# YukunXia/VLOAM-CMU-16833

Measured on AMD Instinct MI355X. Metric: scans/sec end-to-end odometry on 64x2048 cloud, higher is better.
Workload: dtype f32 points / f64 poses+residuals; 1 GPU; configs[2]: scanRegistration + laserOdometry + laserMapping scan-to-map ICP (voxel-hash local map, ~200 scans), synthetic HDL-64E 64x2048; sequences=1, map_warmup_sweeps=200, map_points_at_last_sweep=119454

## Files before the change

vloam-cmu-16833_amd/__init__.py:

```python
import os as _os
_os.environ.setdefault("GPU_MAX_HW_QUEUES", "16")
import ctypes as C
import os
import numpy as np

_DIR = os.path.dirname(os.path.abspath(__file__))
LIB_PATH = os.environ.get("VLOAM_HIP_LIB") or os.path.join(_DIR, "libvloam_hip.so")

VLOAM_OK, ERR_INVALID, ERR_HIP, ERR_CAPACITY, ERR_EMPTY, ERR_NO_DEVICE, ERR_ORDER = 0, -1, -2, -3, -4, -5, -6

K_MAX_RINGS, K_SECTORS = 64, 6
K_MAX_SHARP, K_MAX_LESS_SHARP, K_MAX_FLAT = 768, 7680, 1536
K_MAX_LO_FACTORS = K_MAX_SHARP + K_MAX_FLAT
K_IMG_MAX_CORNERS = 1024
K_LM_MAX_TRACE = 104
K_STACK_CAP_CORNER, K_STACK_CAP_SURF = 8192, 24576
K_MAP_FACTOR_CAP = K_STACK_CAP_CORNER + K_STACK_CAP_SURF


class VloamError(RuntimeError):
    def __init__(self, status, msg):
        super().__init__("vloam status %d: %s" % (status, msg))
        self.status = status

# ... 900 lines not shown
        if q_wmap_wodom is not None:
            opt.q_wmap_wodom[:] = [float(v) for v in q_wmap_wodom]
        if t_wmap_wodom is not None:
            opt.t_wmap_wodom[:] = [float(v) for v in t_wmap_wodom]
        return opt

    @staticmethod
    def _import_result(out):
        return {k: (out[0][k].copy() if out[0][k].ndim else out[0][k].item()) for k in MAP_IMPORT_RESULT_DTYPE.names if k != "pad"}

    def map_import(self, corner, surf, q_wmap_wodom=None, t_wmap_wodom=None):
        opt = self._import_options(q_wmap_wodom, t_wmap_wodom)
        c, s = self._cloud_arg(corner), self._cloud_arg(surf)
        out = np.zeros(1, dtype=MAP_IMPORT_RESULT_DTYPE)
        self._chk(self.L.vloam_map_import(self.h, C.byref(opt), c[1], C.c_longlong(c[2]), s[1], C.c_longlong(s[2]), _fp(out)))
        return self._import_result(out)

    def map_import_device(self, corner, surf, q_wmap_wodom=None, t_wmap_wodom=None):
        import torch
        opt = self._import_options(q_wmap_wodom, t_wmap_wodom)
        ptr, n = [None, None], [0, 0]
        for k, c in enumerate((corner, surf)):
            if c is not None and c.shape[0] > 0:
                assert c.is_cuda and c.is_contiguous() and c.dtype == torch.float32 and c.shape[-1] == 4
                ptr[k], n[k] = C.c_void_p(c.data_ptr()), int(c.shape[0])
        res = torch.zeros(MAP_IMPORT_RESULT_DTYPE.itemsize, dtype=torch.uint8, device=next((c.device for c in (corner, surf) if c is not None), "cuda"))
        self._chk(self.L.vloam_map_import_device(self.h, C.byref(opt), ptr[0], C.c_longlong(n[0]), ptr[1], C.c_longlong(n[1]), C.c_void_p(res.data_ptr())))
        return self._import_result(res.cpu().numpy().view(MAP_IMPORT_RESULT_DTYPE))

    def published_map(self):
        n, f = C.c_longlong(0), C.c_int(-1)
        self._chk(self.L.vloam_get_published_map(self.h, None, C.c_longlong(0), C.byref(n), C.byref(f)))
        buf = np.zeros((max(n.value, 1), 4), dtype=np.float32)
        self._chk(self.L.vloam_get_published_map(self.h, _fp(buf), C.c_longlong(n.value), C.byref(n), C.byref(f)))
        return buf[:n.value], f.value

    def published_cloud(self):
        n, f = C.c_int(0), C.c_int(-1)
        self._chk(self.L.vloam_get_published_cloud(self.h, None, 0, C.byref(n), C.byref(f)))
        buf = np.zeros((max(n.value, 1), 4), dtype=np.float32)
        self._chk(self.L.vloam_get_published_cloud(self.h, _fp(buf), n.value, C.byref(n), C.byref(f)))
        return buf[:n.value], f.value

    def published_device_ptr(self, which):
        p, n, f = C.c_void_p(), C.c_longlong(0), C.c_int(-1)
        self._chk(self.L.vloam_published_device_ptr(self.h, int(which), C.byref(p), C.byref(n), C.byref(f)))
        return p.value, n.value, f.value

    def map_health(self):
        v = self.debug_raw(2, 69, np.int32)
        return dict(keys=(int(v[0]), int(v[4])), purged=(int(v[1]), int(v[5])), block_keys=(int(v[2]), int(v[6])), rebuilds=int(v[8]),
                    max_candidates=int(v[9]), deferred=(int(v[10]), int(v[11])))

    def map_force_rebuild(self):
        n = C.c_longlong(0)
        self._chk(self.L.vloam_debug_get(self.h, 2, 70, None, C.c_longlong(0), C.byref(n)))

    def map_force_grow(self):
        n = C.c_longlong(0)
        self._chk(self.L.vloam_debug_get(self.h, 2, 74, None, C.c_longlong(0), C.byref(n)))

    def map_dump(self, kind):
        rows = self.debug_raw(2, 67 + kind, np.uint32, max_bytes=1 << 30).reshape(-1, 7)
        return rows[:, 2].astype(np.int32), rows[:, 3:7].copy().view(np.float32)


def _same_cloud(given, own):
    a = np.ascontiguousarray(given, dtype=np.float32).reshape(-1, 4)
    return a.shape == own.shape and np.array_equal(a.view(np.uint32), np.ascontiguousarray(own).view(np.uint32))


class ScanRegistration:

    def __init__(self, handle):
        self.hd = handle

    def init(self):
        pass

    def reset(self):
        self.hd.reset_frame()

    def input(self, laserCloudIn):
        self.hd.scan_registration(laserCloudIn)

    def output(self):
        return tuple(self.hd.features(k) for k in range(5))


class LaserOdometry:

    def __init__(self, handle):
        self.hd = handle
        self._pose = None

    def init(self):
        pass

    def input(self, *clouds):
        if not clouds:
            return
        if len(clouds) != 5:
            raise TypeError("LaserOdometry.input takes the five clouds of ScanRegistration.output")
        edits = {}
        for k, (name, c) in enumerate(zip(("laserCloud", "cornerPointsSharp", "cornerPointsLessSharp", "surfPointsFlat", "surfPointsLessFlat"), clouds)):
            if not _same_cloud(c, self.hd.features(k)):
# ... 81 lines not shown
```

vloam-cmu-16833_amd/csrc/map_kernels.h:

```cpp
#pragma once
#include <hip/hip_runtime.h>
#include <vector>
#include "../../include/vloam_hip/c_api.h"
#include "sr_kernels.h"
#include "vloam_device.h"

namespace vloam {

constexpr int kCubeW = 21, kCubeH = 21, kCubeD = 11, kCubeNum = kCubeW * kCubeH * kCubeD;
constexpr int kStackCapCorner = 8192;
constexpr int kStackCapSurf = 24576;
constexpr int kMapFactorCap = kStackCapCorner + kStackCapSurf;
constexpr int kStackCapSurfStep = 8192, kStackCapSurfMax = 131072;
static_assert(kStackCapSurfMax <= (1 << 17), "the tier's raw-point arrival stamp keeps 17 bits of stack index (k_map_finalize_tier)");
constexpr int kPendCap = 16;
__host__ __device__ inline int vox_radix(float inv) { return (int)(50.0f * inv) + 4; }

struct __attribute__((aligned(32))) VoxelRec {
  unsigned long long key;
  float sx, sy, sz, si;
  int count;
  int pend_cnt;
};
static_assert(sizeof(VoxelRec) == 32, "one voxel, one half cache line");

struct VoxelTable {
  VoxelRec* rec;
  int* pend;
  unsigned mask;
  ulonglong2* blk;
  unsigned bslots_mask;
  int* stats;
  __host__ __device__ void rebase(size_t off) { rbp(rec, off); rbp(pend, off); rbp(blk, off); rbp(stats, off); }
};
constexpr int kMaxProbe = 128;
constexpr int kCandChunk = 256;
constexpr int kCandCache = 128;

constexpr int kDsMaxBins = 256;
constexpr int kDsBinTarget = 512;
constexpr int kDsBinCap = 4096;
constexpr int kDsBigCell = 32;
constexpr int kDsBigCap = 128;

struct DsScratch {
  unsigned long long* region;
  unsigned long long* over;
  unsigned long long* tmp;
  unsigned long long* sorted;
  unsigned long long* splitters;
  int* cursor;
  unsigned long long* done;
  int stack_cap;
  __host__ __device__ void rebase(size_t off) {
    rbp(region, off); rbp(over, off); rbp(tmp, off); rbp(sorted, off); rbp(splitters, off); rbp(cursor, off); rbp(done, off);
  }
};

struct StackInfo {
  int n_stack[2];
  int error;
};

struct MapFrame {
  int n_uniq[2];
  int n_stack[2];
  int n_touched[2];
  int n_deferred[2];
  int n_newraw[2];
  int rolled;
  int error;
  int n_factors[2][2];
  int max_candidates;
  int fallback_solves;
};

constexpr int kPubBuckets = 2 * kCubeNum;
constexpr int kPubLdsKeys = 4096;
constexpr long long kPubMapCapDefault = 2097152, kPubMapCapMin = 256, kPubMapCapMax = 16777216;
struct PubHeader { long long n; int overflow; int pad; };
struct MapPub {
  int pub_number = 0;
  int skip_n = 1;
  bool due(int frame_count) const { return ((long long)frame_count * skip_n) % pub_number == 0; }
  long long cap = 0;
  int cloud_on = 0;
  int* cnt = nullptr;
  int* off = nullptr;
  int* cur = nullptr;
  unsigned long long* keys = nullptr;
  float4* vals = nullptr;
  float4* out[2] = {nullptr, nullptr};
  PubHeader* hdr[2] = {nullptr, nullptr};
  float4* cloud[2] = {nullptr, nullptr};
  int* cloud_n[2] = {nullptr, nullptr};
  hipEvent_t ev_map[2] = {nullptr, nullptr}, ev_cloud[2] = {nullptr, nullptr};
  int map_seq = 0, cloud_seq = 0;
  int map_frame[2] = {-1, -1}, cloud_frame[2] = {-1, -1};
  int mapped = 0;
  void rebase(size_t o) {
    rbp(cnt, o); rbp(off, o); rbp(cur, o); rbp(keys, o); rbp(vals, o);
    for (int k = 0; k < 2; k++) { rbp(out[k], o); rbp(hdr[k], o); rbp(cloud[k], o); rbp(cloud_n[k], o); }
  }
};

struct MapGrow {
  int max_log2 = 28;
  int lg[2] = {0, 0};
  long long steps = 0;
  long long inc_rec[2] = {0, 0};
  long long inc_blk[2] = {0, 0};
  unsigned long long* progress = nullptr;
  long long step_at[2] = {-1, -1};
  static constexpr int kEvRing = 4;
  hipEvent_t ev_prog[kEvRing] = {};
  int failed_log2 = 0;
  struct Retired { void* p[3]; hipEvent_t ev; };
  std::vector<Retired> retired;
  std::vector<void*> leftover;
};

struct LocAux { int shift[3]; int si_error; double guess[7]; };
struct MapLocalize {
  char* base = nullptr;
  MapState* state = nullptr;
  MapFrame* frame = nullptr;
  LocAux* aux = nullptr;
// ... 12 lines not shown
};

struct MapContext {
  MapState* state = nullptr;
  MapFrame* frame = nullptr;
  VoxelTable tab[2];
  int* cube_cnt = nullptr;
  DsScratch ds[2];
  unsigned ds_gen = 0;
  static constexpr int kSets = kBufferSets;
  float4* stack_sets[kSets][2] = {};
  StackInfo* stack_info[kSets] = {};
  float4* stack[2] = {nullptr, nullptr};
  float4* stack_map[2] = {nullptr, nullptr};
  int* touched[2] = {nullptr, nullptr};
  int* deferred[2] = {nullptr, nullptr};
  int* newraw[2] = {nullptr, nullptr};
  FactorTable F[2];
  LMRecord* rec = nullptr;
  int surf_cap = kStackCapSurf;
  int factor_cap() const { return kStackCapCorner + surf_cap; }
  bool tier() const { return surf_cap > kStackCapSurf; }
  float4* nbr = nullptr;
  int4* cbox = nullptr;
  float4* ccand = nullptr;
  VoxelRec* rebuild_tmp = nullptr;
  int rebuild_cap = 0;
  int* rebuild_n = nullptr;
  int* host_flags = nullptr;
  int rebuild_cooldown[kMaxBatch][2] = {};
  long long rebuilds = 0;
  MapGrow* grow = nullptr;
  Sess se;
  int sel = 0;
  MapContext for_session(int b) const {
    MapContext m = *this;
    const size_t off = (size_t)b * se.ss;
    rbp(m.state, off); rbp(m.frame, off); m.tab[0].rebase(off); m.tab[1].rebase(off); rbp(m.cube_cnt, off); m.ds[0].rebase(off); m.ds[1].rebase(off);
    for (int c = 0; c < kSets; c++) { rbp(m.stack_sets[c][0], off); rbp(m.stack_sets[c][1], off); rbp(m.stack_info[c], off); }
    for (int k = 0; k < 2; k++) { rbp(m.stack[k], off); rbp(m.stack_map[k], off); rbp(m.touched[k], off); rbp(m.deferred[k], off); rbp(m.newraw[k], off); m.F[k].rebase(off); }
    rbp(m.rec, off); rbp(m.nbr, off); rbp(m.cbox, off); rbp(m.ccand, off); rbp(m.registered, off); rbp(m.assoc_cyc, off); rbp(m.ts_log, off); rbp(m.rebuild_tmp, off); rbp(m.rebuild_n, off);
    if (m.host_flags) m.host_flags += 2 * b;
    m.pub.rebase(off);
    m.se.B = 1; m.sel = 0;
    return m;
  }
  MapLocalize* loc = nullptr;
  MapPub pub;
  float4* registered = nullptr;
  long long* assoc_cyc = nullptr;
  long long* ts_log = nullptr;
  int max_points = 0;
  float inv_leaf[2] = {0, 0};
};

vloam_status map_layout(MapContext* m, const vloam_config& cfg, Arena& A);
vloam_status map_init(MapContext* m, hipStream_t st);
vloam_status map_enqueue(MapContext* m, const vloam_config& cfg, hipStream_t st, const SRBuffers& cur, LOState* lo, double* traj_row14,
                         bool skip_frame, int set, ProfHook* ph, hipEvent_t done = nullptr);
vloam_status map_force_rebuild(MapContext* m, hipStream_t st);
void map_destroy(MapContext* m);
vloam_status map_stack_enqueue(MapContext* m, hipStream_t st, const SRBuffers& cur, int set, ProfHook* ph, hipEvent_t done = nullptr);
vloam_status map_get_cloud(MapContext* m, hipStream_t st, int which, const SRBuffers& cur, float* xyzi4, int cap, int* n);
vloam_status map_export(MapContext* m, hipStream_t st, float* xyzi4, long long cap, long long* n);
vloam_status map_export_kind(MapContext* m, hipStream_t st, int kind, float* xyzi4, long long cap, long long* n);
bool map_publishes(const MapContext* m, bool skip_frame);
vloam_status map_publish_enqueue(MapContext* m, hipStream_t st, const float4* cloud, const FrameScalars* S, int frame, bool skip_frame, ProfHook* ph,
                                 hipEvent_t done);
vloam_status map_published_get(MapContext* m, int which, float* xyzi4, long long cap, long long* n, int* frame, void** d_ptr);
vloam_status map_error(MapContext* m, int* err_bits, int clear_mask = 0, long long* fallback_solves = nullptr);
vloam_status map_debug_get(MapContext* m, int item, void* buf, long long cap, long long* n);
vloam_status map_counts(MapContext* m, long long c[16]);
vloam_status map_query_enqueue(MapContext* m, hipStream_t st, int kind, int k, float radius, const void* d_xyz_pad4, int n, void* d_xyzi4, void* d_d2,
                               void* d_count);
vloam_status map_score_enqueue(MapContext* m, hipStream_t st, const void* d_corner, int n_corner, const void* d_surf, int n_surf, const int stride[2],
                               const float radius[2], const double* d_q4t3, int M, void* d_out);
vloam_status map_localize_alloc(MapContext* m, hipStream_t st);
void map_localize_free(MapContext* m);
vloam_status map_localize_enqueue(MapContext* m, hipStream_t st, const float4* corner, int n_corner, const float4* surf, int n_surf, int set,
                                  const double* row7, const double pose7[7], int pose_frame, vloam_localize_result* d_result);
void map_loc_prepare_launch(hipStream_t st, const MapContext* m, const StackInfo* si, const double* row7, const double pose7[7], int pose_frame);
void map_loc_finish_launch(hipStream_t st, const MapContext* m, vloam_localize_result* d_result);
void map_stack_enqueue_loc(MapContext* m, hipStream_t st, const float4* corner, const float4* surf);
vloam_status map_import_run(MapContext* m, hipStream_t st, const double pose7[7], const void* const cloud[2], const int n[2], bool host_clouds,
                            vloam_map_import_result* h_result);
vloam_status map_force_grow(MapContext* m, hipStream_t st);
void map_grow_release(MapContext* m);
vloam_status map_grow_init(MapContext* m, hipStream_t st);
void map_grow_destroy(MapContext* m);
vloam_status map_grow_rehash(MapContext* m, hipStream_t st, int kind);
vloam_status map_grow_before_sweep(MapContext* m, hipStream_t st);
void map_grow_progress_enqueue(MapContext* m, hipStream_t st);
vloam_status map_ckpt_pack(MapContext* m, hipStream_t st, long long n_rec[2], VoxelRec** d_out, float ms[2]);
vloam_status map_ckpt_unpack(MapContext* m, hipStream_t st, const void* recs, const long long n_rec[2], float* ms);
int map_grow_restore_log2(const MapContext* m, int kind, long long live, long long blk);
vloam_status map_grow_restore(MapContext* m, hipStream_t st, const int lg[2], const long long live[2], const long long blk[2], long long mapped);

}
```

vloam-cmu-16833_amd/csrc/map_kernels.hip:

```cpp
#include <hip/hip_runtime.h>
#include <math.h>
#include <string.h>
#include <type_traits>
#include "lm_solve.h"
#include "map_kernels.h"
#include "map_device.h"
#include "map_table.h"
#include "subwave.h"

namespace vloam {

__device__ void map_purge(const VoxelTable& T, const MapState* ms, int first, int stride) {
  const int cW = ms->cenW, cH = ms->cenH, cD = ms->cenD;
  int dead = 0;
  for (unsigned s = (unsigned)first; s <= T.mask; s += (unsigned)stride) {
    const RecVal v = rec_load(&T.rec[s]);
    if (v.key == 0 || v.count == 0) continue;
    int Ai, Aj, Ak;
    unpack_cube(v.key, &Ai, &Aj, &Ak);
    const int i = Ai + cW, j = Aj + cH, kk = Ak + cD;
    if (i < 0 || i >= kCubeW || j < 0 || j >= kCubeH || kk < 0 || kk >= kCubeD) { rec_store_value(&T.rec[s], make_float4(0.f, 0.f, 0.f, 0.f), 0, 0); dead++; }
  }
  if (dead) atomicAdd(&T.stats[1], dead);
}
// ... 13 lines not shown
  const double emin = q + 2.0 * p * cos(phi + 2.0943951023931954923);
  *e_max = emax;
  *e_mid = 3.0 * q - emax - emin;
  const double r0[3] = {A[0][0] - emax, A[0][1], A[0][2]}, r1[3] = {A[0][1], A[1][1] - emax, A[1][2]}, r2[3] = {A[0][2], A[1][2], A[2][2] - emax};
  const double c0[3] = {r0[1] * r1[2] - r0[2] * r1[1], r0[2] * r1[0] - r0[0] * r1[2], r0[0] * r1[1] - r0[1] * r1[0]};
  const double c1[3] = {r0[1] * r2[2] - r0[2] * r2[1], r0[2] * r2[0] - r0[0] * r2[2], r0[0] * r2[1] - r0[1] * r2[0]};
  const double c2[3] = {r1[1] * r2[2] - r1[2] * r2[1], r1[2] * r2[0] - r1[0] * r2[2], r1[0] * r2[1] - r1[1] * r2[0]};
  const double n0 = c0[0] * c0[0] + c0[1] * c0[1] + c0[2] * c0[2], n1 = c1[0] * c1[0] + c1[1] * c1[1] + c1[2] * c1[2],
               n2 = c2[0] * c2[0] + c2[1] * c2[1] + c2[2] * c2[2];
  const bool u0 = n0 >= n1 && n0 >= n2, u1 = !u0 && n1 >= n2;
  const double nn = u0 ? n0 : (u1 ? n1 : n2);
  const double inv = 1.0 / sqrt(nn);
#pragma unroll
  for (int k = 0; k < 3; k++) v[k] = (u0 ? c0[k] : (u1 ? c1[k] : c2[k])) * inv;
}

__device__ bool householder_ls_5x3(double* A, double* b, double* x) {
  const int m = 5, n = 3;
  for (int k = 0; k < n; k++) {
    double nrm = 0;
    for (int i = k; i < m; i++) nrm += A[i * n + k] * A[i * n + k];
    nrm = sqrt(nrm);
    if (nrm == 0.0) return false;
    const double alpha = (A[k * n + k] > 0) ? -nrm : nrm;
    const double v0 = A[k * n + k] - alpha;
    double vtv = v0 * v0;
    for (int i = k + 1; i < m; i++) vtv += A[i * n + k] * A[i * n + k];
    if (vtv != 0.0) {
      for (int j = k + 1; j < n; j++) {
        double s = v0 * A[k * n + j];
        for (int i = k + 1; i < m; i++) s += A[i * n + k] * A[i * n + j];
        s = 2.0 * s / vtv;
        A[k * n + j] -= s * v0;
        for (int i = k + 1; i < m; i++) A[i * n + j] -= s * A[i * n + k];
      }
      double s = v0 * b[k];
      for (int i = k + 1; i < m; i++) s += A[i * n + k] * b[i];
      s = 2.0 * s / vtv;
      b[k] -= s * v0;
      for (int i = k + 1; i < m; i++) b[i] -= s * A[i * n + k];
    }
    A[k * n + k] = alpha;
    for (int i = k + 1; i < m; i++) A[i * n + k] = 0.0;
  }
  for (int k = n - 1; k >= 0; k--) {
    double s = b[k];
    for (int j = k + 1; j < n; j++) s -= A[k * n + j] * x[j];
    if (A[k * n + k] == 0.0) return false;
    x[k] = s / A[k * n + k];
  }
  return true;
}

template <int G, int KB>
__global__ __launch_bounds__(256) __attribute__((amdgpu_waves_per_eu(5))) void k_map_assoc(const float4* __restrict__ stack0, const float4* __restrict__ stack1, VoxelTable T0,
                                                   VoxelTable T1, float inv0, float inv1, const MapState* __restrict__ ms, MapFrame* fr,
                                                   float4* __restrict__ nbr, int outer, int4* __restrict__ cbox, float4* __restrict__ ccand,
                                                   long long* __restrict__ dbg_cyc , size_t ss) {
  VL_SESSION(ss); RB(stack0); RB(stack1); T0.rebase(so_); T1.rebase(so_); RB(ms); RB(fr); RB(nbr); RB(cbox); RB(ccand); RB(dbg_cyc);
  long long tp[8] = {0, 0, 0, 0, 0, 0, 0, 0};
  if (dbg_cyc) tp[0] = clock64();
  constexpr int Q = 64 / G, QW = 4 * Q;
  constexpr int U = G == 16 ? 4 : 2, CH = U * G;
  static_assert(CH <= kCandCache, "the second round's candidate cache holds kCandCache entries per slot");
  const int lane = threadIdx.x & 63, wave = threadIdx.x >> 6, gl = lane & (G - 1), qi = wave * Q + lane / G;
  const int nc = ms->n_corner_stack, nsf = ms->n_surf_stack;
  const int wc = (nc + QW - 1) / QW, ws = (nsf + QW - 1) / QW, cpc = (wc + 7) >> 3, cps = (ws + 7) >> 3;
  const int bq = (int)blockIdx.x >> 3, xcd = (int)blockIdx.x & 7;
  if (bq >= cpc + cps || !ms->do_optimize) return;
  const int kind = bq < cpc ? 0 : 1;
  const int i = (kind ? xcd * cps + (bq - cpc) : xcd * cpc + bq) * QW + qi;
  const bool live = i < (kind ? nsf : nc);
  if (__ballot(live) == 0ull) return;
  const int slot = kind ? kStackCapCorner + i : i;
  const VoxelTable T = kind ? T1 : T0;
  const float inv = kind ? inv1 : inv0;
  const unsigned nv = (unsigned)vox_radix(inv);
  __shared__ u64 s_cand[QW][CH + 8];
  __shared__ u64 s_bestk[QW][8];
  __shared__ float4 s_bestp[QW][8];
  __shared__ int s_piece[QW][3][8];
  __shared__ int s_np[QW][4];
  constexpr int kRawCap = 64;
  __shared__ u64 s_rawk[QW][kRawCap];
  __shared__ int s_rawn[QW][kRawCap];
  __shared__ int s_nraw[QW];
  float4 pointOri = make_float4(0.f, 0.f, 0.f, 0.f);
  int4 box0 = make_int4(0, 0, 0, 0), box1 = make_int4(0, 0, -1, 0);
  if (live) {
    pointOri = kind ? stack1[i] : stack0[i];
    if (outer > 0) { box0 = cbox[2 * slot]; box1 = cbox[2 * slot + 1]; }
  }
  const float4 sel = associate_to_map(pointOri, ms->parameters, ms->parameters + 4);
  const float q0 = sel.x, q1 = sel.y, q2 = sel.z;
  const int cen0 = ms->cenW, cen1 = ms->cenH, cen2 = ms->cenD;
  const int ctr0 = ms->centerCube[0] - cen0, ctr1 = ms->centerCube[1] - cen1, ctr2 = ms->centerCube[2] - cen2;
  const float mg = outer == 0 ? 1.051f : 1.001f;
  int blo0 = (int)floorf((q0 - mg) * inv), bhi0 = (int)floorf((q0 + mg) * inv);
  int blo1 = (int)floorf((q1 - mg) * inv), bhi1 = (int)floorf((q1 + mg) * inv);
  int blo2 = (int)floorf((q2 - mg) * inv), bhi2 = (int)floorf((q2 + mg) * inv);
  bool from_cache = false;
  int total = 0;
  if (outer > 0 && live) {
    const int4 b0 = box0, b1 = box1;
    from_cache = b1.z >= 0 && b1.z <= kCandCache && b0.x <= blo0 && b0.y >= bhi0 && b0.z <= blo1 && b0.w >= bhi1 && b1.x <= blo2 && b1.y >= bhi2;
    if (from_cache) total = b1.z;
  }
  const bool search = live && !from_cache;
  bool chain_too_long = false;
  if (dbg_cyc) tp[1] = clock64() + (__float_as_int(q0) & 0) + (total & 0);
  if (gl < 8) s_bestk[qi][gl] = ~0ull;
  if (gl < 4) s_np[qi][gl] = 0;
  if (gl == 4) s_nraw[qi] = 0;
  sw_lds_sync();
  if (__ballot(search) != 0ull) {
    if (search && gl < 3) {
      const int lo = gl == 0 ? blo0 : (gl == 1 ? blo1 : blo2), hi = gl == 0 ? bhi0 : (gl == 1 ? bhi1 : bhi2);
      const int ctr = gl == 0 ? ctr0 : (gl == 1 ? ctr1 : ctr2), cen = gl == 0 ? cen0 : (gl == 1 ? cen1 : cen2);
      const int halfw = gl == 2 ? 1 : 2, wdim = gl == 0 ? kCubeW : (gl == 1 ? kCubeH : kCubeD);
      const double leaf = 1.0 / (double)inv;
      const int Amin = cube_lo((double)lo * leaf), Amax = cube_hi((double)(hi + 1) * leaf);
      int n = 0;
      bool ovf = false;
      for (int A = Amin; A <= Amax; A++) {
        if (abs(A - ctr) > halfw) continue;
        const int wv = A + cen;
        if (wv < 0 || wv >= wdim) continue;
        const int base = cube_voxel_base(A, inv);
        const int ia = max(lo, base + 1), ib = min(hi, cube_voxel_base(A + 1, inv) + 1);
        if (ia > ib) continue;
        for (int blk = (ia - base) >> 2; blk <= ((ib - base) >> 2); blk++) {
          if ((unsigned)blk > (unsigned)(kVoxMax >> 2) || n >= 8) { ovf = true; break; }
          int m4 = 0;
#pragma unroll
          for (int t = 0; t < 4; t++) { const int iv = base + (blk << 2) + t; if (iv >= ia && iv <= ib) m4 |= 1 << t; }
          s_piece[qi][gl][n] = ((A + 8192) << 11) | (blk << 4) | m4;
          n++;
        }
      }
      s_np[qi][gl] = n;
      if (ovf) s_np[qi][3] = 1;
    }
    sw_lds_sync();
  }
// ... 167 lines not shown
    }
    if (__ballot(from_cache && act) != 0ull) {
      float4 cc[U];
#pragma unroll
      for (int u = 0; u < U; u++) {
        const int w = c0 + gl + u * G;
        cc[u] = make_float4(0.f, 0.f, 0.f, __uint_as_float(0xffffffffu));
        if (from_cache && act && w < total) cc[u] = ccand[(size_t)slot * kCandCache + w];
      }
#pragma unroll
      for (int u = 0; u < U; u++) {
        const unsigned tie = __float_as_uint(cc[u].w);
        const float d0 = q0 - cc[u].x, d1 = q1 - cc[u].y, d2 = q2 - cc[u].z;
        const u64 k = ((u64)__float_as_uint(d0 * d0 + d1 * d1 + d2 * d2) << 32) | tie;
        if (from_cache && tie != 0xffffffffu) { key_u[u] = k; px[u] = cc[u].x; py[u] = cc[u].y; pz[u] = cc[u].z; }
      }
    }
    if (dbg_cyc && c0 == 0) tp[4] = clock64() + ((int)key_u[0] & 0);
    select_rounds(act, c0 > 0);
    if (dbg_cyc && c0 == 0) tp[5] = clock64();
  }
  const int nraw = min(s_nraw[qi], kRawCap);
  const bool raw_overflow = s_nraw[qi] > kRawCap;
  if (__ballot(live && nraw > 0) != 0ull) {
    int total_raw = 0;
    for (c0 = 0;; c0 += CH) {
      const bool act = live && nraw > 0 && (c0 == 0 || c0 < total_raw);
      if (__ballot(act) == 0ull) break;
      reset_candidates();
      int produced = 0;
      for (int r0 = 0; __ballot(act && r0 < nraw) != 0ull; r0 += G) {
        const int r = r0 + gl;
        const int nr = (act && r < nraw) ? s_rawn[qi][r] : 0;
        const u64 vk = (act && r < nraw) ? s_rawk[qi][r] : 0ull;
        const int inc = grp_scan_incl<G>(nr);
        const int tot = grp_sum<G>(nr);
        int o = produced + inc - nr;
        for (int j = 1; j <= nr; j++, o++)
          if (o >= c0 && o < c0 + CH) s_cand[qi][o - c0] = key_with_seq(vk, j);
        produced += tot;
      }
      if (act) total_raw = produced;
      sw_lds_sync();
      ncand = act ? min(total_raw - c0, CH) : 0;
      probe_pair(std::integral_constant<int, 0>{});
      if constexpr (U > 2) { if (__ballot(2 * G < ncand) != 0ull) probe_pair(std::integral_constant<int, 2>{}); }
      select_rounds(act, true);
    }
  }
  if (outer == 0 && search && gl == 0) {
    cbox[2 * slot] = make_int4(blo0, bhi0, blo1, bhi1);
    cbox[2 * slot + 1] = make_int4(blo2, bhi2, (total <= kCandCache && !overflow && s_nraw[qi] == 0) ? total : -1, total);
  }
  if (live && gl < 5) {
    const u64 k4 = s_bestk[qi][4];
    const bool ok = k4 != ~0ull && __uint_as_float((unsigned)(k4 >> 32)) < 1.0f;
    float4 p = s_bestp[qi][gl];
    p.w = ok ? 1.0f : 0.0f;
    nbr[slot * 5 + gl] = p;
  }
  if (live && gl == 0 && total > kCandChunk) atomicMax(&fr->max_candidates, total);
  if (__ballot(chain_too_long || (live && overflow)) && lane == 0) atomicOr(&fr->error, kErrMapFull);
  if (__ballot(live && raw_overflow) && lane == 0) atomicOr(&fr->error, kErrMapDeferred);
  if (dbg_cyc && lane == 0) {
    tp[6] = clock64();
    if (tp[3] == 0) tp[3] = tp[2];
    if (tp[4] == 0) tp[4] = tp[3];
    for (int k = 0; k < 6; k++) atomicAdd((unsigned long long*)&dbg_cyc[outer * 8 + k], (unsigned long long)(tp[k + 1] - tp[k]));
    atomicAdd((unsigned long long*)&dbg_cyc[outer * 8 + 7], 1ull);
  }
}

#define VL_MAP_TIER 0
#define VL_MAP_KERNEL(name) name
#define VL_MAP_CAP_PARAM
#define VL_MAP_SURF_CAP kStackCapSurf
#define VL_MAP_FACTOR_CAP kMapFactorCap
#include "map_prepare_fit.inc.h"
#define VL_MAP_TIER 1
#define VL_MAP_KERNEL(name) name##_tier
#define VL_MAP_CAP_PARAM , int surf_cap
#define VL_MAP_SURF_CAP surf_cap
#define VL_MAP_FACTOR_CAP F.cap
#include "map_prepare_fit.inc.h"

__device__ void map_update(MapState* ms, double* traj_row14) {
  const double* q = ms->q_wodom_curr;
  const double n2 = q[0] * q[0] + q[1] * q[1] + q[2] * q[2] + q[3] * q[3];
  double qi[4] = {0, 0, 0, 0};
  if (n2 > 0.0) { qi[0] = -q[0] / n2; qi[1] = -q[1] / n2; qi[2] = -q[2] / n2; qi[3] = q[3] / n2; }
  double r[4], t[3];
  dquat_mul(ms->parameters, qi, r);
  for (int k = 0; k < 4; k++) ms->q_wmap_wodom[k] = r[k];
  dquat_rot(ms->q_wmap_wodom, ms->t_wodom_curr, t);
  for (int k = 0; k < 3; k++) ms->t_wmap_wodom[k] = ms->parameters[4 + k] - t[k];
  if (traj_row14) for (int k = 0; k < 7; k++) traj_row14[7 + k] = ms->parameters[k];
}

__device__ bool map_put_raw_point(const VoxelTable& T, u64 voxel_key, int seq, float4 p, int stamp) {
  const u64 key = key_with_seq(voxel_key, seq);
  unsigned s = (unsigned)mix64(key) & T.mask;
  for (int probe = 0; probe < kMaxProbe; probe++, s = (s + 1) & T.mask) {
    const u64 old = atomicCAS(&T.rec[s].key, 0ull, key);
    if (old == 0ull || old == key) {
      if (old == 0ull) atomicAdd(&T.stats[0], 1);
      rec_store_value(&T.rec[s], p, 1, stamp);
      return true;
    }
  }
  return false;
}
__device__ void map_drop_raw_points(const VoxelTable& T, u64 voxel_key, int n) {
// ... 252 lines not shown
}

vloam_status map_layout(MapContext* m, const vloam_config& cfg, Arena& A) {
  bool ok = true;
  ok = ok && A.take(&m->state, 1) && A.take(&m->frame, 1) && A.take(&m->cube_cnt, 2 * (size_t)kCubeNum);
  const int lg = cfg.map_capacity_log2 < 10 ? 10 : (cfg.map_capacity_log2 > 28 ? 28 : cfg.map_capacity_log2);
  const size_t slots = (size_t)1 << lg;
  for (int k = 0; k < 2 && ok; k++) {
    VoxelTable& T = m->tab[k];
    if (m->grow) { T.rec = nullptr; T.pend = nullptr; T.blk = nullptr; ok = ok && A.take(&T.stats, 4); }
    else ok = ok && A.take(&T.rec, slots) && A.take(&T.pend, slots * kPendCap) && A.take(&T.stats, 4);
    T.mask = (unsigned)(slots - 1);
    const size_t bslots = slots / 2;
    if (!m->grow) ok = ok && A.take(&T.blk, bslots);
    T.bslots_mask = (unsigned)(bslots - 1);
    DsScratch& D = m->ds[k];
    if (k == 0) for (int c = 0; c < MapContext::kSets; c++) ok = ok && A.take(&m->stack_info[c], 1);
    D.stack_cap = k ? m->surf_cap : kStackCapCorner;
    ok = ok && A.take(&D.region, (size_t)kDsMaxBins * kDsBinCap) && A.take(&D.over, (size_t)cfg.max_points) && A.take(&D.tmp, (size_t)cfg.max_points) &&
         A.take(&D.sorted, (size_t)cfg.max_points) && A.take(&D.splitters, (size_t)kDsMaxBins) && A.take(&D.cursor, (size_t)kDsMaxBins + 4) &&
         A.take(&D.done, (size_t)kDsMaxBins);
    for (int c = 0; c < MapContext::kSets; c++) ok = ok && A.take(&m->stack_sets[c][k], (size_t)D.stack_cap);
    m->stack[k] = m->stack_sets[0][k];
    ok = ok && A.take(&m->stack_map[k], (size_t)D.stack_cap) && A.take(&m->touched[k], (size_t)D.stack_cap) && A.take(&m->deferred[k], (size_t)D.stack_cap) &&
         A.take(&m->newraw[k], (size_t)D.stack_cap);
    FactorTable& F = m->F[k];
    F.cap = m->factor_cap();
    ok = ok && A.take(&F.type, (size_t)F.cap) && A.take(&F.p, 3 * (size_t)F.cap) && A.take(&F.A, 3 * (size_t)F.cap) && A.take(&F.B, 3 * (size_t)F.cap) &&
         A.take(&F.resid, 3 * (size_t)F.cap) && A.take(&F.ctype, (size_t)F.cap) && A.take(&F.cslot, (size_t)F.cap) && A.take(&F.cpack, 11 * (size_t)F.cap) && A.take(&F.dg, 8 * (size_t)F.cap) &&
         A.take(&F.rowcnt, (size_t)F.cap / 64 + 1);
    if (m->tier()) F.rowmask = nullptr;
    else ok = ok && A.take(&F.rowmask, (size_t)F.cap / 64 + 2);
    F.gsync = nullptr;
    F.err = ok ? &m->frame->error : nullptr;
    F.fallbacks = ok ? &m->frame->fallback_solves : nullptr;
    F.host_degraded = nullptr;
    F.gen = 0; F.spin_limit = 1 << 18;
  }
  ok = ok && A.take(&m->rec, 2) && A.take(&m->nbr, 5 * (size_t)m->factor_cap());
  ok = ok && A.take(&m->cbox, 2 * (size_t)m->factor_cap()) && A.take(&m->ccand, (size_t)m->factor_cap() * kCandCache);
  m->rebuild_cap = m->grow ? 0 : (int)(slots / 2);
  if (m->grow) { m->rebuild_tmp = nullptr; m->grow->lg[0] = m->grow->lg[1] = lg; ok = ok && A.take(&m->rebuild_n, 2); }
  else ok = ok && A.take(&m->rebuild_tmp, (size_t)m->rebuild_cap) && A.take(&m->rebuild_n, 2);
  ok = ok && A.take(&m->registered, (size_t)cfg.max_points) && A.take(&m->assoc_cyc, 16) && A.take(&m->ts_log, 2048);
  MapPub& P = m->pub;
  if (P.pub_number > 0) {
    ok = ok && A.take(&P.cnt, (size_t)kPubBuckets) && A.take(&P.off, (size_t)kPubBuckets + 1) && A.take(&P.cur, (size_t)kPubBuckets) &&
         A.take(&P.keys, (size_t)P.cap) && A.take(&P.vals, (size_t)P.cap);
    for (int k = 0; k < 2; k++) ok = ok && A.take(&P.out[k], (size_t)P.cap) && A.take(&P.hdr[k], 1);
  }
  if (P.cloud_on) for (int k = 0; k < 2; k++) ok = ok && A.take(&P.cloud[k], (size_t)cfg.max_points) && A.take(&P.cloud_n[k], 1);
  if (!ok) return VLOAM_ERR_HIP;
  m->max_points = cfg.max_points;
  m->inv_leaf[0] = 1.0f / cfg.mapping_line_resolution;
  m->inv_leaf[1] = 1.0f / cfg.mapping_plane_resolution;
  return VLOAM_OK;
}

vloam_status map_init(MapContext* m, hipStream_t st) {
  if (m->grow && map_grow_init(m, st) != VLOAM_OK) return VLOAM_ERR_HIP;
  if (!m->host_flags) {
    if (hipHostMalloc((void**)&m->host_flags, sizeof(int) * 2 * kMaxBatch, hipHostMallocMapped) != hipSuccess) { m->host_flags = nullptr; return VLOAM_ERR_HIP; }
    for (int k = 0; k < 2 * kMaxBatch; k++) m->host_flags[k] = 0;
  }
  for (int k = 0; k < 2; k++) {
    if (m->pub.pub_number > 0 && !m->pub.ev_map[k] && hipEventCreateWithFlags(&m->pub.ev_map[k], hipEventDisableTiming | hipEventBlockingSync) != hipSuccess) return VLOAM_ERR_HIP;
    if (m->pub.cloud_on && !m->pub.ev_cloud[k] && hipEventCreateWithFlags(&m->pub.ev_cloud[k], hipEventDisableTiming | hipEventBlockingSync) != hipSuccess) return VLOAM_ERR_HIP;
  }
  MapState init;
  memset(&init, 0, sizeof(init));
  init.parameters[3] = 1.0; init.q_wmap_wodom[3] = 1.0; init.q_wodom_curr[3] = 1.0;
  init.cenW = 10; init.cenH = 10; init.cenD = 5;
  if (hipMemcpyAsync(m->state, &init, sizeof(init), hipMemcpyHostToDevice, st) != hipSuccess) return VLOAM_ERR_HIP;
  return hipStreamSynchronize(st) == hipSuccess ? VLOAM_OK : VLOAM_ERR_HIP;
}

void map_destroy(MapContext* m) {
  map_localize_free(m);
  if (m->grow) map_grow_destroy(m);
  if (m->host_flags) { (void)hipHostFree(m->host_flags); m->host_flags = nullptr; }
  for (int k = 0; k < 2; k++)
    for (hipEvent_t* e : {&m->pub.ev_map[k], &m->pub.ev_cloud[k]}) if (*e) { (void)hipEventDestroy(*e); *e = nullptr; }
}

static vloam_status map_rebuild_enqueue(MapContext* m0, hipStream_t st, int session, int kind) {
  if (m0->grow) return map_grow_rehash(m0, st, kind);
  MapContext ms_ = m0->for_session(session);
  MapContext* m = &ms_;
  VoxelTable& T = m->tab[kind];
  const size_t slots = (size_t)T.mask + 1, bslots = (size_t)T.bslots_mask + 1;
  const int cap = kind ? m->surf_cap : kStackCapCorner;
  if (hipMemsetAsync(m->rebuild_n, 0, sizeof(int), st) != hipSuccess) return VLOAM_ERR_HIP;
  VL_RAW_LAUNCH(k_map_rebuild_gather, dim3(1024), dim3(256), 0, st, T, m->rebuild_tmp, m->rebuild_cap, m->rebuild_n, m->frame, kind);
  if (hipMemsetAsync(T.rec, 0, slots * sizeof(VoxelRec), st) != hipSuccess) return VLOAM_ERR_HIP;
  if (hipMemsetAsync(T.blk, 0, bslots * sizeof(ulonglong2), st) != hipSuccess) return VLOAM_ERR_HIP;
  if (hipMemsetAsync(T.stats, 0, 4 * sizeof(int), st) != hipSuccess) return VLOAM_ERR_HIP;
  VL_RAW_LAUNCH(k_map_rebuild_insert, dim3(1024), dim3(256), 0, st, T, m->rebuild_tmp, m->rebuild_cap, m->rebuild_n, m->frame, kind,
                     m->deferred[kind], cap, m->inv_leaf[kind], m->host_flags);
  m0->rebuilds++;
  return hipGetLastError() == hipSuccess ? VLOAM_OK : VLOAM_ERR_HIP;
}

vloam_status map_force_rebuild(MapContext* m, hipStream_t st) {
  for (int b = 0; b < m->se.B; b++)
    for (int k = 0; k < 2; k++) { vloam_status s = map_rebuild_enqueue(m, st, b, k); if (s != VLOAM_OK) return s; }
  return VLOAM_OK;
}

static const bool g_ts_log = getenv("VLOAM_TS_LOG") != nullptr;
vloam_status map_enqueue(MapContext* m, const vloam_config& cfg, hipStream_t st, const SRBuffers& cur, LOState* lo, double* traj_row14,
                         bool skip_frame, int set, ProfHook* ph, hipEvent_t done) {
  (void)cur;
  MapState* ms = m->state;
  MapFrame* fr = m->frame;
  const unsigned Z = (unsigned)m->se.B;
  const size_t ss = m->se.ss;
  m->stack[0] = m->stack_sets[set][0]; m->stack[1] = m->stack_sets[set][1];
  if (m->grow && !skip_frame && map_grow_before_sweep(m, st) != VLOAM_OK) return VLOAM_ERR_HIP;
  if (!skip_frame) {
    for (int b = 0; b < m->se.B; b++)
      for (int k = 0; k < 2; k++) {
        if (m->rebuild_cooldown[b][k] > 0) { m->rebuild_cooldown[b][k]--; continue; }
        if (__atomic_load_n(&m->host_flags[2 * b + k], __ATOMIC_RELAXED)) {
          if (map_rebuild_enqueue(m, st, b, k) != VLOAM_OK) return VLOAM_ERR_HIP;
          m->rebuild_cooldown[b][k] = 8;
        }
      }
  }
  const bool tier = m->tier();
  const int S = m->surf_cap;
#define VL_PREPARE(KERN, ...)                                                                                                                          \
  VLOAM_LAUNCH_EV(ph, kKMapPrepare, st, skip_frame ? done : nullptr, KERN, dim3(1, 1, Z), dim3(256), 0, st, ms, fr, lo, m->cube_cnt, skip_frame ? 1 : 0, \
                  traj_row14, m->stack_info[set], m->deferred[0], m->deferred[1], m->newraw[0], m->newraw[1], g_ts_log ? m->ts_log : (long long*)nullptr, __VA_ARGS__)
  if (tier) VL_PREPARE(k_map_prepare_tier, ss, S);
  else VL_PREPARE(k_map_prepare, ss);
#undef VL_PREPARE
  if (skip_frame) return hipGetLastError() == hipSuccess ? VLOAM_OK : VLOAM_ERR_HIP;
  m->pub.mapped++;
  for (int outer = 0; outer < 2; outer++) {
    static const int g_env = getenv("VLOAM_MAP_ASSOC_LANES") ? atoi(getenv("VLOAM_MAP_ASSOC_LANES")) : -1;
    const int G = g_env >= 0 ? g_env : (m->se.B > 1 ? 16 : 32);
    auto grid_for = [S](int g) { const int qw = 256 / g; return dim3(8 * ((kStackCapCorner / qw + 7) / 8 + (S / qw + 7) / 8), 1, 1); };
#define VL_MAP_ASSOC(KERN, GRID)                                                                                                      \
    VLOAM_LAUNCH(ph, kKMapAssoc, st, KERN, dim3((GRID).x, 1, Z), dim3(256), 0, st, m->stack[0], m->stack[1], m->tab[0], m->tab[1], \
                 m->inv_leaf[0], m->inv_leaf[1], ms, fr, m->nbr, outer, m->cbox, m->ccand, cfg.debug ? m->assoc_cyc : (long long*)nullptr, ss)
    static const int kb_env = getenv("VLOAM_MAP_ASSOC_KB") ? atoi(getenv("VLOAM_MAP_ASSOC_KB")) : 2;
    if (G == 16 && kb_env == 1) VL_MAP_ASSOC((k_map_assoc<16, 1>), grid_for(16));
    else if (G == 16) VL_MAP_ASSOC((k_map_assoc<16, 2>), grid_for(16));
    else if (G == 64) VL_MAP_ASSOC((k_map_assoc<64, 1>), grid_for(64));
    else VL_MAP_ASSOC((k_map_assoc<32, 1>), grid_for(32));
#undef VL_MAP_ASSOC
#define VL_FIT(KERN, GRID_X)                                                                                                               \
    VLOAM_LAUNCH(ph, kKMapFit, st, KERN, dim3((GRID_X), 1, Z), dim3(256), 0, st, m->stack[0], m->stack[1], m->tab[0], m->tab[1], ms, fr, m->nbr, \
                 m->F[outer], outer, ss)
    if (tier) VL_FIT(k_map_fit_tier, m->factor_cap() / 256);
    else VL_FIT(k_map_fit, kMapFactorCap / 256);
#undef VL_FIT
    lm_launch(st, m->se, m->F[outer], kStackCapCorner, ms->parameters, m->rec + outer, 4, 0.1, true, &ms->do_optimize, ph);
  }
#define VL_INSERT(KERN, ...)                                                                                                                  \
  VLOAM_LAUNCH(ph, kKMapInsert, st, KERN, dim3(64, 2, Z), dim3(256), 0, st, m->stack[0], m->stack[1], m->stack_map[0], m->stack_map[1], m->tab[0], \
               m->tab[1], m->inv_leaf[0], m->inv_leaf[1], ms, fr, m->touched[0], m->touched[1], m->deferred[0], m->deferred[1], traj_row14, __VA_ARGS__)
#define VL_FINALIZE(KERN, GRID_X, ...)                                                                                                           \
  VLOAM_LAUNCH_EV(ph, kKMapFinalize, st, done, KERN, dim3((GRID_X), 2, Z), dim3(256), 0, st, m->stack_map[0], m->stack_map[1], m->tab[0], m->tab[1], \
                  ms, fr, m->touched[0], m->touched[1], m->deferred[0], m->deferred[1], m->newraw[0], m->newraw[1], m->cube_cnt, m->host_flags,      \
                  g_ts_log ? m->ts_log : (long long*)nullptr, __VA_ARGS__)
  if (tier) { VL_INSERT(k_map_insert_tier, ss, S); VL_FINALIZE(k_map_finalize_tier, S / 256, ss, S); }
  else { VL_INSERT(k_map_insert, ss); VL_FINALIZE(k_map_finalize, kStackCapSurf / 256, ss); }
#undef VL_INSERT
#undef VL_FINALIZE
  if (m->grow) map_grow_progress_enqueue(m, st);
  return hipGetLastError() == hipSuccess ? VLOAM_OK : VLOAM_ERR_HIP;
}

vloam_status map_localize_enqueue(MapContext* m, hipStream_t st, const float4* corner, int n_corner, const float4* surf, int n_surf, int set,
                                  const double* row7, const double pose7[7], int pose_frame, vloam_localize_result* d_result) {
  MapLocalize* L = m->loc;
  const float4* stack[2] = {m->stack_sets[set][0], m->stack_sets[set][1]};
  const StackInfo* si = m->stack_info[set];
  if (corner || surf) {
    SRBuffers b{};
    b.S = L->S; b.less_sharp = const_cast<float4*>(corner); b.less_flat = const_cast<float4*>(surf);
    if (hipMemsetAsync(L->si, 0, sizeof(StackInfo), st) != hipSuccess) return VLOAM_ERR_HIP;
    sr_adopt_launch(st, b, -1, -1, n_corner, -1, n_surf);
    map_stack_enqueue_loc(m, st, corner, surf);
    stack[0] = L->stack[0]; stack[1] = L->stack[1];
    si = L->si;
  }
  map_loc_prepare_launch(st, m, si, row7, pose7, pose_frame);
  MapState* ms = L->state;
  MapFrame* fr = L->frame;
  Sess se = m->se;
  se.B = 1; se.ss = 0;
  for (int outer = 0; outer < 2; outer++) {
    const int qw = 256 / 32;
    VL_RAW_LAUNCH((k_map_assoc<32, 1>), dim3(8 * ((kStackCapCorner / qw + 7) / 8 + (kStackCapSurf / qw + 7) / 8), 1, 1), dim3(256), 0, st, stack[0], stack[1],
                  m->tab[0], m->tab[1], m->inv_leaf[0], m->inv_leaf[1], ms, fr, L->nbr, outer, L->cbox, L->ccand, (long long*)nullptr, (size_t)0);
    VL_RAW_LAUNCH(k_map_fit, dim3(kMapFactorCap / 256, 1, 1), dim3(256), 0, st, stack[0], stack[1], m->tab[0], m->tab[1], ms, fr, L->nbr, L->F[outer], outer,
                  (size_t)0);
    lm_launch(st, se, L->F[outer], kStackCapCorner, ms->parameters, L->rec + outer, 4, 0.1, true, &ms->do_optimize, nullptr);
  }
  map_loc_finish_launch(st, m, d_result);
  return hipGetLastError() == hipSuccess ? VLOAM_OK : VLOAM_ERR_HIP;
}

}
```

Baseline: 6751 scans/s.

## Fuse second-round map fit into association kernel and reuse unchanged neighbor factors

On the second outer ICP round, the association kernel now also fits line and plane factors directly, so the separate k_map_fit launch is skipped. When a query's five nearest neighbors match the previous round bit-for-bit, the earlier factor (A, B, digest) is copied instead of recomputed. Unserved factor slots are cleared inside the same kernel. This removes one launch and a reread of the neighbor buffer, but adds register and LDS pressure plus a block-wide sync to the already heavy association kernel. It runs only for G=32, non-tier, unless the env var VLOAM_MAP_ROUND2_PAIR is set.

```diff
diff --git a/vloam-cmu-16833_amd/__init__.py b/vloam-cmu-16833_amd/__init__.py
--- a/vloam-cmu-16833_amd/__init__.py
+++ b/vloam-cmu-16833_amd/__init__.py
@@ -976,6 +976,10 @@
         return dict(keys=(int(v[0]), int(v[4])), purged=(int(v[1]), int(v[5])), block_keys=(int(v[2]), int(v[6])), rebuilds=int(v[8]),
                     max_candidates=int(v[9]), deferred=(int(v[10]), int(v[11])))
 
+    def map_round2_counts(self):
+        v = self.debug_raw(2, 65, np.int32)
+        return dict(reused=int(v[18]), refit=int(v[19]), searched=int(v[20]))
+
     def map_force_rebuild(self):
         n = C.c_longlong(0)
         self._chk(self.L.vloam_debug_get(self.h, 2, 70, None, C.c_longlong(0), C.byref(n)))
diff --git a/vloam-cmu-16833_amd/csrc/map_kernels.h b/vloam-cmu-16833_amd/csrc/map_kernels.h
--- a/vloam-cmu-16833_amd/csrc/map_kernels.h
+++ b/vloam-cmu-16833_amd/csrc/map_kernels.h
@@ -73,6 +73,7 @@
   int n_factors[2][2];
   int max_candidates;
   int fallback_solves;
+  int round2[3];
 };
 
 constexpr int kPubBuckets = 2 * kCubeNum;
@@ -191,6 +192,7 @@
   long long* ts_log = nullptr;
   int max_points = 0;
   float inv_leaf[2] = {0, 0};
+  bool round2_pair = false;
 };
 
 vloam_status map_layout(MapContext* m, const vloam_config& cfg, Arena& A);
diff --git a/vloam-cmu-16833_amd/csrc/map_kernels.hip b/vloam-cmu-16833_amd/csrc/map_kernels.hip
--- a/vloam-cmu-16833_amd/csrc/map_kernels.hip
+++ b/vloam-cmu-16833_amd/csrc/map_kernels.hip
@@ -89,11 +89,59 @@
   return true;
 }
 
-template <int G, int KB>
+__device__ __forceinline__ int map_fit_five(int kind, const float4* nb, double (&A3)[3], double (&B3)[3]) {
+  int type = 0;
+  if (kind == 0) {
+    double center[3] = {0, 0, 0};
+#pragma unroll
+    for (int j = 0; j < 5; j++) { const float4 p = nb[j]; center[0] = center[0] + (double)p.x; center[1] = center[1] + (double)p.y; center[2] = center[2] + (double)p.z; }
+    for (int a = 0; a < 3; a++) center[a] = center[a] / 5.0;
+    double cov[3][3] = {{0, 0, 0}, {0, 0, 0}, {0, 0, 0}};
+#pragma unroll
+    for (int j = 0; j < 5; j++) {
+      const float4 p = nb[j];
+      const double z[3] = {(double)p.x - center[0], (double)p.y - center[1], (double)p.z - center[2]};
+      for (int a = 0; a < 3; a++) for (int b = 0; b < 3; b++) cov[a][b] = cov[a][b] + z[a] * z[b];
+    }
+    double e_mid, e_max, dir[3];
+    sym_eig3_top(cov, &e_mid, &e_max, dir);
+    if (e_max > 3 * e_mid) {
+      for (int a = 0; a < 3; a++) { A3[a] = 0.1 * dir[a] + center[a]; B3[a] = -0.1 * dir[a] + center[a]; }
+      type = 1;
+    }
+  } else {
+    double matA0[15], matB0[5], nrm[3];
+#pragma unroll
+    for (int j = 0; j < 5; j++) { const float4 p = nb[j]; matA0[j * 3] = p.x; matA0[j * 3 + 1] = p.y; matA0[j * 3 + 2] = p.z; matB0[j] = -1.0; }
+    if (householder_ls_5x3(matA0, matB0, nrm)) {
+      const double nn_ = sqrt(nrm[0] * nrm[0] + nrm[1] * nrm[1] + nrm[2] * nrm[2]);
+      const double negative_OA_dot_norm = 1 / nn_;
+      nrm[0] = nrm[0] / nn_; nrm[1] = nrm[1] / nn_; nrm[2] = nrm[2] / nn_;
+      bool planeValid = true;
+      sw_lds_sync();
+#pragma unroll
+      for (int j = 0; j < 5; j++) {
+        const float4 p = nb[j];
+        if (fabs(nrm[0] * (double)p.x + nrm[1] * (double)p.y + nrm[2] * (double)p.z + negative_OA_dot_norm) > 0.2) planeValid = false;
+      }
+      if (planeValid) { A3[0] = nrm[0]; A3[1] = nrm[1]; A3[2] = nrm[2]; B3[0] = negative_OA_dot_norm; type = 3; }
+    }
+  }
+  return type;
+}
+
+struct Round2Tables {
+  FactorTable F0, F1;
+  int* counts;
+};
+template <class T> __device__ __forceinline__ const T& round2_tables(const T& t) { return t; }
+
+template <int G, int KB, bool R2 = false, class... R2Args>
 __global__ __launch_bounds__(256) __attribute__((amdgpu_waves_per_eu(5))) void k_map_assoc(const float4* __restrict__ stack0, const float4* __restrict__ stack1, VoxelTable T0,
                                                    VoxelTable T1, float inv0, float inv1, const MapState* __restrict__ ms, MapFrame* fr,
                                                    float4* __restrict__ nbr, int outer, int4* __restrict__ cbox, float4* __restrict__ ccand,
-                                                   long long* __restrict__ dbg_cyc , size_t ss) {
+                                                   long long* __restrict__ dbg_cyc , size_t ss, R2Args... r2) {
+  static_assert(sizeof...(R2Args) == (R2 ? 1 : 0), "the fused second round takes one Round2Tables");
   VL_SESSION(ss); RB(stack0); RB(stack1); T0.rebase(so_); T1.rebase(so_); RB(ms); RB(fr); RB(nbr); RB(cbox); RB(ccand); RB(dbg_cyc);
   long long tp[8] = {0, 0, 0, 0, 0, 0, 0, 0};
   if (dbg_cyc) tp[0] = clock64();
@@ -104,11 +152,26 @@
   const int nc = ms->n_corner_stack, nsf = ms->n_surf_stack;
   const int wc = (nc + QW - 1) / QW, ws = (nsf + QW - 1) / QW, cpc = (wc + 7) >> 3, cps = (ws + 7) >> 3;
   const int bq = (int)blockIdx.x >> 3, xcd = (int)blockIdx.x & 7;
+  [[maybe_unused]] FactorTable F0{}, F1{};
+  [[maybe_unused]] int* r2_counts = nullptr;
+  if constexpr (R2) {
+    static_assert(QW == 8, "a workgroup's queries are one byte of a row mask");
+    const Round2Tables& R = round2_tables(r2...);
+    F0 = R.F0; F1 = R.F1; r2_counts = R.counts;
+    F0.rebase(so_); F1.rebase(so_); RB(r2_counts);
+    const int served0 = ms->do_optimize ? 8 * cpc : 0, served1 = ms->do_optimize ? 8 * cps : 0;
+    for (int c = (int)blockIdx.x; c < F1.cap / QW; c += (int)gridDim.x) {
+      const int ck = c < kStackCapCorner / QW ? 0 : 1;
+      if ((ck ? c - kStackCapCorner / QW : c) < (ck ? served1 : served0)) continue;
+      if (threadIdx.x < QW) F1.type[c * QW + threadIdx.x] = 0;
+      if (threadIdx.x == 0) reinterpret_cast<unsigned char*>(F1.rowmask)[c] = 0;
+    }
+  }
   if (bq >= cpc + cps || !ms->do_optimize) return;
   const int kind = bq < cpc ? 0 : 1;
   const int i = (kind ? xcd * cps + (bq - cpc) : xcd * cpc + bq) * QW + qi;
   const bool live = i < (kind ? nsf : nc);
-  if (__ballot(live) == 0ull) return;
+  if constexpr (!R2) { if (__ballot(live) == 0ull) return; }
   const int slot = kind ? kStackCapCorner + i : i;
   const VoxelTable T = kind ? T1 : T0;
   const float inv = kind ? inv1 : inv0;
@@ -127,6 +190,12 @@
   if (live) {
     pointOri = kind ? stack1[i] : stack0[i];
     if (outer > 0) { box0 = cbox[2 * slot]; box1 = cbox[2 * slot + 1]; }
+  }
+  [[maybe_unused]] float4 prev = make_float4(0.f, 0.f, 0.f, 0.f);
+  [[maybe_unused]] int type0 = 0;
+  if constexpr (R2) {
+    if (live && gl < 5) prev = nbr[slot * 5 + gl];
+    if (live) type0 = F0.type[slot];
   }
   const float4 sel = associate_to_map(pointOri, ms->parameters, ms->parameters + 4);
   const float q0 = sel.x, q1 = sel.y, q2 = sel.z;
@@ -400,12 +469,57 @@
     cbox[2 * slot] = make_int4(blo0, bhi0, blo1, bhi1);
     cbox[2 * slot + 1] = make_int4(blo2, bhi2, (total <= kCandCache && !overflow && s_nraw[qi] == 0) ? total : -1, total);
   }
+  [[maybe_unused]] bool same_nbr = false;
   if (live && gl < 5) {
     const u64 k4 = s_bestk[qi][4];
     const bool ok = k4 != ~0ull && __uint_as_float((unsigned)(k4 >> 32)) < 1.0f;
     float4 p = s_bestp[qi][gl];
     p.w = ok ? 1.0f : 0.0f;
     nbr[slot * 5 + gl] = p;
+    if constexpr (R2) same_nbr = __float_as_uint(p.x) == __float_as_uint(prev.x) && __float_as_uint(p.y) == __float_as_uint(prev.y) && __float_as_uint(p.z) == __float_as_uint(prev.z);
+  }
+  if constexpr (R2) {
+    __shared__ int s_accept[QW];
+    const int g0 = lane & ~(G - 1);
+    const bool same5 = ((__ballot(same_nbr) >> g0) & 31ull) == 31ull;
+    const bool ok1 = ((__ballot(gl == 0 && prev.w != 0.0f) >> g0) & 1ull) != 0ull;
+    const u64 k4 = s_bestk[qi][4];
+    const bool fit = live && k4 != ~0ull && __uint_as_float((unsigned)(k4 >> 32)) < 1.0f;
+    const bool reuse = fit && ok1 && same5;
+    const int cap = F1.cap;
+    int type = reuse ? type0 : 0;
+    if (reuse && type0) {
+      const int ndg = F1.dg ? (type0 == 1 ? 8 : 4) : 0;
+      if (gl < 3) F1.A[gl * cap + slot] = F0.A[gl * cap + slot];
+      if (gl >= 3 && gl < 6) F1.B[(gl - 3) * cap + slot] = F0.B[(gl - 3) * cap + slot];
+      if (gl >= 6 && gl < 6 + ndg) F1.dg[(gl - 6) * cap + slot] = F0.dg[(gl - 6) * cap + slot];
+      if (gl == 14) F1.p[slot] = pointOri.x;
+      if (gl == 15) F1.p[cap + slot] = pointOri.y;
+      if (gl == 16) F1.p[2 * cap + slot] = pointOri.z;
+    }
+    if (fit && !reuse && gl == 0) {
+      double A3[3] = {0, 0, 0}, B3[3] = {0, 0, 0};
+      type = map_fit_five(kind, s_bestp[qi], A3, B3);
+      if (type) {
+        F1.p[slot] = pointOri.x; F1.p[cap + slot] = pointOri.y; F1.p[2 * cap + slot] = pointOri.z;
+        F1.A[slot] = A3[0]; F1.A[cap + slot] = A3[1]; F1.A[2 * cap + slot] = A3[2];
+        F1.B[slot] = B3[0]; F1.B[cap + slot] = B3[1]; F1.B[2 * cap + slot] = B3[2];
+        factor_digest(F1, slot, type, A3, B3);
+      }
+    }
+    if (gl == 0) { F1.type[slot] = type; s_accept[qi] = type != 0 ? 1 : 0; }
+    if (r2_counts) {
+      const u64 b0 = __ballot(gl == 0 && reuse), b1 = __ballot(gl == 0 && fit && !reuse), b2 = __ballot(gl == 0 && search);
+      if (lane == 0) { if (b0) atomicAdd(&r2_counts[0], __popcll(b0)); if (b1) atomicAdd(&r2_counts[1], __popcll(b1)); if (b2) atomicAdd(&r2_counts[2], __popcll(b2)); }
+    }
+    __syncthreads();
+    if (threadIdx.x == 0) {
+      int m = 0;
+#pragma unroll
+      for (int q = 0; q < QW; q++) m |= s_accept[q] << q;
+      reinterpret_cast<unsigned char*>(F1.rowmask)[slot / QW] = (unsigned char)m;
+      if (m) atomicAdd(&fr->n_factors[outer][kind], __popc(m));
+    }
   }
   if (live && gl == 0 && total > kCandChunk) atomicMax(&fr->max_candidates, total);
   if (__ballot(chain_too_long || (live && overflow)) && lane == 0) atomicOr(&fr->error, kErrMapFull);
@@ -764,6 +878,7 @@
   if (P.cloud_on) for (int k = 0; k < 2; k++) ok = ok && A.take(&P.cloud[k], (size_t)cfg.max_points) && A.take(&P.cloud_n[k], 1);
   if (!ok) return VLOAM_ERR_HIP;
   m->max_points = cfg.max_points;
+  { const char* e = getenv("VLOAM_MAP_ROUND2_PAIR"); m->round2_pair = e && atoi(e) != 0; }
   m->inv_leaf[0] = 1.0f / cfg.mapping_line_resolution;
   m->inv_leaf[1] = 1.0f / cfg.mapping_plane_resolution;
   return VLOAM_OK;
@@ -857,7 +972,13 @@
     VLOAM_LAUNCH(ph, kKMapAssoc, st, KERN, dim3((GRID).x, 1, Z), dim3(256), 0, st, m->stack[0], m->stack[1], m->tab[0], m->tab[1], \
                  m->inv_leaf[0], m->inv_leaf[1], ms, fr, m->nbr, outer, m->cbox, m->ccand, cfg.debug ? m->assoc_cyc : (long long*)nullptr, ss)
     static const int kb_env = getenv("VLOAM_MAP_ASSOC_KB") ? atoi(getenv("VLOAM_MAP_ASSOC_KB")) : 2;
-    if (G == 16 && kb_env == 1) VL_MAP_ASSOC((k_map_assoc<16, 1>), grid_for(16));
+    const bool fused = outer == 1 && G != 16 && G != 64 && !tier && !m->round2_pair;
+    if (fused) {
+      const Round2Tables r2{m->F[0], m->F[1], cfg.debug ? &fr->round2[0] : (int*)nullptr};
+      VLOAM_LAUNCH(ph, kKMapAssoc, st, (k_map_assoc<32, 1, true, Round2Tables>), dim3(grid_for(32).x, 1, Z), dim3(256), 0, st, m->stack[0], m->stack[1], m->tab[0],
+                   m->tab[1], m->inv_leaf[0], m->inv_leaf[1], ms, fr, m->nbr, outer, m->cbox, m->ccand, cfg.debug ? m->assoc_cyc : (long long*)nullptr, ss, r2);
+    }
+    else if (G == 16 && kb_env == 1) VL_MAP_ASSOC((k_map_assoc<16, 1>), grid_for(16));
     else if (G == 16) VL_MAP_ASSOC((k_map_assoc<16, 2>), grid_for(16));
     else if (G == 64) VL_MAP_ASSOC((k_map_assoc<64, 1>), grid_for(64));
     else VL_MAP_ASSOC((k_map_assoc<32, 1>), grid_for(32));
@@ -865,7 +986,8 @@
 #define VL_FIT(KERN, GRID_X)                                                                                                               \
     VLOAM_LAUNCH(ph, kKMapFit, st, KERN, dim3((GRID_X), 1, Z), dim3(256), 0, st, m->stack[0], m->stack[1], m->tab[0], m->tab[1], ms, fr, m->nbr, \
                  m->F[outer], outer, ss)
-    if (tier) VL_FIT(k_map_fit_tier, m->factor_cap() / 256);
+    if (fused) {}
+    else if (tier) VL_FIT(k_map_fit_tier, m->factor_cap() / 256);
     else VL_FIT(k_map_fit, kMapFactorCap / 256);
 #undef VL_FIT
     lm_launch(st, m->se, m->F[outer], kStackCapCorner, ms->parameters, m->rec + outer, 4, 0.1, true, &ms->do_optimize, ph);
```

Result: slower. 6426 scans/s (-4.8%).
